# Codeuser0717/CVAE-GAN

Hardware: NVIDIA B200
Metric: train_samples_per_s (higher is better)
Workload: dtype f32

## Files before the change

cvae_gan_b200/csrc/api.cu:

```cuda
#include "engine.cuh"

namespace cvg {
const char* last_error();
int comm_unique_id(void* out128);
int comm_init(Engine& e, const void* id128, int rank, int world);
void comm_destroy(Engine& e);
}

using namespace cvg;

struct CvgHandle {
  Engine e;
};

#define H_OR_FAIL(h)                      \
  if (!(h)) {                             \
    cvg::set_error("null handle");        \
    return 1;                             \
  }


constexpr int FC_MAX_KC = 12;
template <int KC>
struct FcDispatch {
// ... 182 lines not shown

int cvg_nvl_local_handle(CvgHandle* h, void* out64) {
  H_OR_FAIL(h);
  if (!out64) CVG_FAIL("null argument");
  return nvl_local_handle(h->e, out64);
}
int cvg_nvl_attach(CvgHandle* h, const void* handles) {
  H_OR_FAIL(h);
  if (!handles) CVG_FAIL("null argument");
  return nvl_attach(h->e, handles);
}

int cvg_nvl_disable(CvgHandle* h) {
  H_OR_FAIL(h);
  nvl_destroy(h->e);
  return 0;
}

int cvg_step_d(CvgHandle* h, const float* x_real, int label, int B, const CvgNoise* noise, uint64_t seed,
               uint64_t counter, int flags, float* loss_out, void* stream) {
  H_OR_FAIL(h);
  if (!x_real) CVG_FAIL("null x_real");
  if (label < 0 || label >= h->e.K) CVG_FAIL("label out of range");
  StepRng rng;
  rng.seed = seed; rng.counter = counter;
  return step_d(h->e, x_real, label, B, noise, rng, flags, loss_out, (cudaStream_t)stream);
}
int cvg_step_c(CvgHandle* h, const float* x_real, int label, int B, const CvgNoise* noise, uint64_t seed,
               uint64_t counter, int flags, float* loss_out, void* stream) {
  H_OR_FAIL(h);
  if (!x_real) CVG_FAIL("null x_real");
  if (label < 0 || label >= h->e.K) CVG_FAIL("label out of range");
  StepRng rng;
  rng.seed = seed; rng.counter = counter;
  return step_c(h->e, x_real, label, B, noise, rng, flags, loss_out, (cudaStream_t)stream);
}
int cvg_step_g(CvgHandle* h, const float* x_real, int label, int B, const CvgNoise* noise, uint64_t seed,
               uint64_t counter, float lambda_class_now, int flags, float* loss_out, void* stream) {
  H_OR_FAIL(h);
  if (!x_real && !(flags & CVG_STEP_PRIOR_ONLY)) CVG_FAIL("null x_real");
  if ((flags & CVG_STEP_PRIOR_ONLY) && (flags & CVG_STEP_CVAE)) CVG_FAIL("CVG_STEP_PRIOR_ONLY and CVG_STEP_CVAE are mutually exclusive");
  if (label < 0 || label >= h->e.K) CVG_FAIL("label out of range");
  StepRng rng;
  rng.seed = seed; rng.counter = counter;
  rng.lambda_class = lambda_class_now; rng.lambda_nonzero = lambda_class_now != 0.f;
  return step_g(h->e, x_real, label, B, noise, rng, flags, loss_out, (cudaStream_t)stream);
}

int cvg_step_classifier(CvgHandle* h, const float* x, const int64_t* labels, int B, const CvgNoise* noise, uint64_t seed,
                        uint64_t counter, float lr, float beta1, float beta2, float eps, int flags, float* loss_out,
                        void* stream) {
  H_OR_FAIL(h);
  if (!x || !labels) CVG_FAIL("cvg_step_classifier: null argument");
  StepRng rng;
  rng.seed = seed; rng.counter = counter;
  AdamOverride ov{lr, beta1, beta2, eps};
  return step_classifier(h->e, x, (const long long*)labels, B, noise, rng, ov, flags, loss_out, (cudaStream_t)stream);
}

int cvg_visit(CvgHandle* h, int label, int B_local, int64_t B_global, const float* class_rows, int64_t n_rows,
              const float* x_batches, int d_loop, int c_loop, int g_loop, int flags, float* loss_out, void* stream) {
  H_OR_FAIL(h);
  if (label < 0 || label >= h->e.K) CVG_FAIL("label out of range");
  if (d_loop < 0 || c_loop < 0 || g_loop < 0) CVG_FAIL("cvg_visit: negative loop count");
  if ((flags & CVG_STEP_PRIOR_ONLY) && (flags & CVG_STEP_CVAE)) CVG_FAIL("CVG_STEP_PRIOR_ONLY and CVG_STEP_CVAE are mutually exclusive");
  if ((flags & CVG_STEP_CVAE) && d_loop != 0) CVG_FAIL("cvg_visit: a CVAE visit has no critic steps (d_loop must be 0, cvae.py:86-166)");
  return visit(h->e, label, B_local, B_global, class_rows, n_rows, x_batches, d_loop, c_loop, g_loop, flags, loss_out,
               (cudaStream_t)stream);
}

int cvg_ctl_set(CvgHandle* h, uint64_t seed, uint64_t counter, int set_rng, float lambda_class, int set_lambda, void* stream) {
  H_OR_FAIL(h);
  if (!h->e.ws_base) CVG_FAIL("workspace not bound");
  ctl_set_kernel<<<1, 32, 0, (cudaStream_t)stream>>>(h->e.ws.ctl, seed, counter, set_rng, lambda_class, set_lambda);
  CVG_CUDA(cudaGetLastError());
  h->e.launches++;
  return 0;
}

int cvg_adam(CvgHandle* h, int net_mask, void* stream) {
  H_OR_FAIL(h);
  return run_adam(h->e, net_mask, (cudaStream_t)stream);
}

int cvg_sample_rows(CvgHandle* h, const float* class_rows, int64_t n, int64_t B_global, int64_t draw_offset,
                    int B_local, uint64_t seed, uint64_t counter, float* x_out, int64_t* idx_out, void* stream) {
  H_OR_FAIL(h);
  if (!class_rows || !x_out || n < 1 || B_local < 1 || draw_offset < 0 || draw_offset + B_local > B_global)
    CVG_FAIL("cvg_sample_rows: bad argument");
  sample_rows_kernel<<<(B_local + 127) / 128, 128, 0, (cudaStream_t)stream>>>(
      class_rows, n, B_global, draw_offset, B_local, h->e.F, seed, counter, nullptr, 0, x_out, (long long*)idx_out);
  CVG_CUDA(cudaGetLastError());
  h->e.launches++;
  return 0;
}

int cvg_generate(CvgHandle* h, int label, int64_t n, const float* z, uint64_t seed, uint64_t row_offset, int train_mode,
                 float* x_out, void* stream) {
  H_OR_FAIL(h);
  if (n < 0 || (n > 0 && !x_out)) CVG_FAIL("cvg_generate: bad argument");
  return generate(h->e, label, n, z, seed, row_offset, train_mode, x_out, (cudaStream_t)stream);
}

int cvg_generate_filter(CvgHandle* h, int label, int64_t n, float thr, const float* z, uint64_t seed,
                        uint64_t row_offset, float* x_out, int64_t* idx_out, int64_t capacity,
                        unsigned long long* count_out, float* logits_out, uint8_t* keep_out, void* stream) {
  H_OR_FAIL(h);
  if (n < 0 || !count_out || (capacity > 0 && !x_out)) CVG_FAIL("cvg_generate_filter: bad argument");
  return generate_filter(h->e, label, n, thr, z, seed, row_offset, x_out, idx_out, capacity, count_out, logits_out,
                         keep_out, (cudaStream_t)stream);
}

int cvg_filter_logits(const float* logits, int64_t n, int K, int label, float thr, uint8_t* keep_out, void* stream) {
  if (!logits || !keep_out || n < 0) CVG_FAIL("cvg_filter_logits: bad argument");
  if (K < 1 || K > FILTER_MAXK) CVG_FAIL("cvg_filter_logits: K must be in [1, 32]");
  if (n == 0) return 0;
  filter_logits_kernel<<<(unsigned)((n + 255) / 256), 256, 0, (cudaStream_t)stream>>>(logits, n, K, label, thr, keep_out);
  CVG_CUDA(cudaGetLastError());
  return 0;
}

int cvg_filter_compact(const float* x, const float* logits, int64_t n, int F, int K, int label, float thr,
                       uint64_t row_offset, float* x_out, int64_t* idx_out, int64_t capacity,
                       unsigned long long* count_out, void* stream) {
  if (!x || !logits || !count_out || n < 0) CVG_FAIL("cvg_filter_compact: bad argument");
  if (K < 1 || K > FILTER_MAXK) CVG_FAIL("cvg_filter_compact: K must be in [1, 32]");
  if (n == 0) return 0;
  if (K > FC_MAX_KC) {
    filter_compact_kernel<false><<<(unsigned)((n + 255) / 256), 256, 0, (cudaStream_t)stream>>>(
        x, logits, n, 0, F, K, label, thr, row_offset, x_out, (long long*)idx_out, capacity, count_out, nullptr, nullptr);
  } else {
    const size_t smem = (size_t)FC_SUB_ROWS * K * sizeof(float);
    static int sms = 0;
    if (!sms) {
      int dev = 0;
      CVG_CUDA(cudaGetDevice(&dev));
      CVG_CUDA(cudaDeviceGetAttribute(&sms, cudaDevAttrMultiProcessorCount, dev));
      CVG_TRY(fc_set_attributes());
    }
    const long long slots = (long long)sms * 6;
    long long done = 0;
    while (done < n) {
      const long long left = n - done;
      const long long nblk1k = (left + FC_SUB_ROWS - 1) / FC_SUB_ROWS;
      const long long grid = nblk1k < slots ? nblk1k : slots;
      long long nsub = (nblk1k + grid - 1) / grid;
      long long rows_now = left;
      if (nsub > FC_MAXSUB) {
        nsub = FC_MAXSUB;
        rows_now = grid * nsub * FC_SUB_ROWS;
      }
      CVG_TRY(fc_launch(K, (unsigned)grid, smem, (cudaStream_t)stream, x + done * F, logits + done * K, rows_now, F, label, thr,
                        row_offset + (uint64_t)done, (int)nsub, x_out, (long long*)idx_out, capacity, count_out));
      CVG_CUDA(cudaGetLastError());
      done += rows_now;
    }
  }
  CVG_CUDA(cudaGetLastError());
  return 0;
}

int cvg_classifier_forward(CvgHandle* h, const float* x, int64_t n, float* logits_out, void* stream) {
  H_OR_FAIL(h);
  if (!x || !logits_out || n < 0) CVG_FAIL("cvg_classifier_forward: bad argument");
  return classifier_forward(h->e, x, n, logits_out, (cudaStream_t)stream);
}
int cvg_encoder_forward(CvgHandle* h, const float* x, int label, int64_t n, float* mu_out, float* logvar_out,
                        void* stream) {
  H_OR_FAIL(h);
  if (!x || !mu_out || !logvar_out || n < 0) CVG_FAIL("cvg_encoder_forward: bad argument");
  return encoder_forward(h->e, x, label, n, mu_out, logvar_out, (cudaStream_t)stream);
}

int cvg_patience_scan(const uint8_t* keep, int64_t n, int64_t num, int chunk, int patience, int64_t* rows_consumed,
                      int64_t* rows_accepted) {
  if (!keep || !rows_consumed || !rows_accepted || chunk < 1) CVG_FAIL("cvg_patience_scan: bad argument");
  int64_t pos = 0, got = 0;
  while (got < num && patience > 0) {
    const int64_t c = (num - got) < chunk ? (num - got) : chunk;
    if (pos + c > n) CVG_FAIL("cvg_patience_scan: row stream too short");
    int64_t k = 0;
    for (int64_t i = 0; i < c; ++i) k += keep[pos + i] ? 1 : 0;
    pos += c;
    got += k;
    if (k == 0) --patience;
  }
  *rows_consumed = pos;
  *rows_accepted = got;
  return 0;
}

int cvg_debug_read(CvgHandle* h, const char* name, int pass, int rows, float* dst, int* features_out, void* stream) {
  H_OR_FAIL(h);
  if (!name) CVG_FAIL("null name");
  Engine& e = h->e;
  const Workspace& w = e.ws;
  if (!e.ws_base) CVG_FAIL("workspace not bound");
  const std::string n(name);
  const float* p = nullptr;
  int C = 0;
  auto idx = [&](const char* prefix) -> int {
    const size_t L = strlen(prefix);
    if (n.size() == L + 1 && n.compare(0, L, prefix) == 0 && n[L] >= '0' && n[L] <= '2') return n[L] - '0';
    return -1;
  };
  int i;
  if (n == "xT") { p = w.xT; C = e.F; }
  else if (n == "z") { p = w.z; C = e.Z; }
  else if ((i = idx("g_h")) >= 0) { p = w.g_h[i]; C = e.gh[i]; }
  else if ((i = idx("g_dy")) >= 0) { p = w.g_dy[i]; C = e.gh[i]; }
  else if (n == "g_out") { p = w.g_out; C = e.F; }
  else if (n == "g_dout") { p = w.g_dout; C = e.F; }
  else if ((i = idx("e_h")) >= 0) { p = w.e_h[i]; C = e.eh[i]; }
  else if ((i = idx("e_dy")) >= 0) { p = w.e_dy[i]; C = e.eh[i]; }
  else if (n == "e_ml") { p = w.e_ml; C = 2 * e.Z; }
  else if (n == "e_dml") { p = w.e_dml; C = 2 * e.Z; }
  else if ((i = idx("d_a")) >= 0) { p = w.d_a[i]; C = e.dh[i]; }
  else if ((i = idx("d_g")) >= 0) { p = w.d_g[i]; C = e.dh[i]; }
  else if (n == "d_s") { p = w.d_s; C = 1; }
  else if (n == "c_a1") { p = w.c_a1; C = e.ch[0]; }
  else if (n == "c_h2") { p = w.c_h2; C = e.ch[1]; }
  else if (n == "c_a2") { p = w.c_a2; C = e.ch[1]; }
  else if (n == "c_a3") { p = w.c_a3; C = e.ch[2]; }
  else if (n == "c_logit") { p = w.c_logit; C = e.K; }
  else if (n == "c_dlogit") { p = w.c_dlogit; C = e.K; }
  else if ((i = idx("c_g")) >= 0) { p = w.c_g[i]; C = e.ch[i]; }
  else if (n == "dx") { p = w.dx; C = e.F; }
  else CVG_FAIL("cvg_debug_read: unknown buffer name");
  if (features_out) *features_out = C;
  if (!dst) return 0;
  if (rows < 1 || rows > w.ld || pass < 0 || pass > 1) CVG_FAIL("cvg_debug_read: bad rows/pass");
  to_row_major_kernel<<<(rows + 127) / 128, 128, 0, (cudaStream_t)stream>>>(p + (size_t)pass * C * w.ld, rows, C, w.ld, dst);
  CVG_CUDA(cudaGetLastError());
  return 0;
}

int cvg_debug_tc_counters(CvgHandle* h, long long* dev_counters) {
  H_OR_FAIL(h);
  h->e.tc_dbg = dev_counters;
  return 0;
}

int cvg_profile_enable(CvgHandle* h, int enable) {
  H_OR_FAIL(h);
  Engine& e = h->e;
  for (auto& r : e.prof_recs) {
    cudaEventDestroy(r.a);
    cudaEventDestroy(r.b);
  }
  e.prof_recs.clear();
  e.prof = enable != 0;
  return 0;
}

int cvg_profile_read(CvgHandle* h, int kernel_class, int64_t* launches, double* flops, double* ms) {
  H_OR_FAIL(h);
  if (!launches || !flops || !ms) CVG_FAIL("cvg_profile_read: null argument");
  Engine& e = h->e;
  *launches = 0;
  *flops = 0.0;
  *ms = 0.0;
  for (auto& r : e.prof_recs) {
    if (r.cls != kernel_class) continue;
    CVG_CUDA(cudaEventSynchronize(r.b));
    float t = 0.f;
    CVG_CUDA(cudaEventElapsedTime(&t, r.a, r.b));
    *launches += 1;
    *flops += r.flops;
    *ms += (double)t;
  }
  return 0;
}

int64_t cvg_launch_count(const CvgHandle* h) { return h ? h->e.launches : -1; }

int cvg_debug_set(CvgHandle* h, const char* key, int value) {
  H_OR_FAIL(h);
  if (!key) CVG_FAIL("null key");
  Engine& e = h->e;
  const std::string k(key);
  if (k == "train_mode") {
    if (value && !mk_supported(e)) CVG_FAIL("cvg_debug_set: the step-program kernel does not cover these layer widths");
    e.mk.enabled = value != 0;
  } else if (k == "mk_max_ops") e.mk.max_ops = value;
  else if (k == "mk_allbar") e.mk.allbar = value != 0;
  else if (k == "mk_coop") e.mk.coop = value != 0;
  else if (k == "hoist") e.hoist = value != 0;
  else if (k == "streams") e.ms.on = value != 0;
  else if (k == "chain") e.chain = value != 0;
  else if (k == "eg_split") e.eg_split = value != 0;
  else if (k == "fuse_stats") e.nvl.fuse = value != 0;
  else CVG_FAIL("cvg_debug_set: unknown key");
  return 0;
}

int cvg_debug_get(const CvgHandle* h, const char* key, int* value) {
  H_OR_FAIL(h);
  if (!key || !value) CVG_FAIL("null argument");
  const Engine& e = h->e;
  const std::string k(key);
  if (k == "train_mode") *value = e.mk.enabled ? 1 : 0;
  else if (k == "mk_last_nops") *value = e.mk.last_nops;
  else if (k == "mk_supported") *value = mk_supported(e) ? 1 : 0;
  else CVG_FAIL("cvg_debug_get: unknown key");
  return 0;
}

int cvg_debug_mk_cycles(CvgHandle* h, long long* out, int capacity, int* count) {
  H_OR_FAIL(h);
  Engine& e = h->e;
  if (!e.ws_base) CVG_FAIL("workspace not bound");
  const int n = e.mk.last_nops < capacity ? e.mk.last_nops : capacity;
  if (count) *count = n;
  if (out && n > 0) CVG_CUDA(cudaMemcpy(out, e.ws.mk_dbg, sizeof(long long) * n, cudaMemcpyDeviceToHost));
  if (out && capacity >= 2048 + 64 && n <= 1024) {
    CVG_CUDA(cudaMemcpy(out + 1024, e.ws.mk_dbg + 1024, sizeof(long long) * n, cudaMemcpyDeviceToHost));
    if (capacity >= 4096)
      for (int i = 0; i < n && i < (int)e.mk.last_kinds.size(); ++i) out[3072 + i] = e.mk.last_kinds[i];
  }
  if (out && capacity >= 2048 + 64) CVG_CUDA(cudaMemcpy(out + 2048, e.ws.mk_dbg + 2048, sizeof(long long) * 64, cudaMemcpyDeviceToHost));
  return 0;
}

}
```

cvae_gan_b200/csrc/chain.cuh:

```cuda
#pragma once
#include "gemm.cuh"
#include "misc_kernels.cuh"

namespace cvg {

constexpr int CH_TM = 32;
constexpr int CH_THREADS = 256;
constexpr int CH_NB = 64;
constexpr int CH_KC = 64;
constexpr int CH_H0 = 256, CH_H1 = 128, CH_H2 = 64;
constexpr int CH_MAX_IN = 256;
constexpr int CH_MAX_K = 32;
constexpr int CH_WBUF = 2 * CH_KC * CH_NB;

struct CriticChainArgs {
  int M = 0, ld = 0, F = 0;
  const float* x = nullptr;
  long long sx = 0;
  const float* W[4] = {};
  int ldw[4] = {};
  const float* b[4] = {};
  const float* wlabel = nullptr;
  int ldwl = 0;
  const float* inv_sigma = nullptr;
  const uint8_t* m1 = nullptr;
  const uint8_t* m2 = nullptr;
  float keep_inv = 1.f, slope = 0.2f;
  float* a[3] = {};
  float* s = nullptr;
  float* g[3] = {};
  double* osum = nullptr;
  float seed[2] = {0.f, 0.f};
};

struct ClassifierChainArgs {
  int M = 0, ld = 0, F = 0, K = 0, label = 0;
  const float* x = nullptr;
  long long sx = 0;
  const float* W[4] = {};
  const float* b[4] = {};
  const float* gamma = nullptr;
  const float* beta = nullptr;
  float ln_eps = 1e-5f;
  const uint8_t* m1 = nullptr;
  const uint8_t* m2 = nullptr;
  float keep_inv = 1.f;
  float *a1 = nullptr, *h2 = nullptr, *a2 = nullptr, *rs = nullptr, *a3 = nullptr, *logit = nullptr, *dlogit = nullptr;
  float* g[3] = {};
  float coef = 1.f;
  double* loss = nullptr;
  float* dgamma = nullptr;
  float* dbeta = nullptr;
  unsigned long long* acc = nullptr;
  unsigned* cnt = nullptr;
};

template <bool WT, class Ep>
__device__ __forceinline__ void chain_layer(const float* X, const float* __restrict__ W, int ldw, int R, int N, float* wbuf,
                                            Ep ep) {
  const int tid = threadIdx.x;
  const int grp = tid >> 6, t64 = tid & 63;
  const int tm = (t64 & 7) * 4, tn = (t64 >> 3) * 8;
  const int Rp = (R + TBK - 1) / TBK * TBK;
  const int nkc = (Rp + CH_KC - 1) / CH_KC;
  const bool wvec = (ldw & 3) == 0;
  for (int n0 = 0; n0 < N; n0 += CH_NB) {
    float4 pre[4];
    auto gload = [&](int kc) {
#pragma unroll
      for (int j = 0; j < 4; ++j) pre[j] = make_float4(0.f, 0.f, 0.f, 0.f);
      if (WT) {
        const int n = n0 + (tid & 63);
        if (n >= N) return;
#pragma unroll
        for (int j = 0; j < 4; ++j) {
          const int k = kc + (tid >> 6) * 16 + 4 * j;
          const float* src = W + (size_t)n * ldw + k;
          if (wvec && k + 3 < R) {
            pre[j] = ld4(src);
          } else {
            if (k < R) pre[j].x = src[0];
            if (k + 1 < R) pre[j].y = src[1];
            if (k + 2 < R) pre[j].z = src[2];
            if (k + 3 < R) pre[j].w = src[3];
          }
        }
      } else {
        const int k = kc + (tid >> 2);
        if (k >= R) return;
#pragma unroll
        for (int j = 0; j < 4; ++j) {
          const int n = n0 + (tid & 3) * 16 + 4 * j;
          const float* src = W + (size_t)k * ldw + n;
          if (wvec && n + 3 < N) {
            pre[j] = ld4(src);
          } else {
            if (n < N) pre[j].x = src[0];
            if (n + 1 < N) pre[j].y = src[1];
            if (n + 2 < N) pre[j].z = src[2];
            if (n + 3 < N) pre[j].w = src[3];
          }
        }
      }
    };
    auto sstore = [&](float* buf) {
      if (WT) {
        const int kq = (tid >> 6) * 16, n = tid & 63;
#pragma unroll
        for (int j = 0; j < 4; ++j) {
          buf[(kq + 4 * j + 0) * CH_NB + n] = pre[j].x;
          buf[(kq + 4 * j + 1) * CH_NB + n] = pre[j].y;
          buf[(kq + 4 * j + 2) * CH_NB + n] = pre[j].z;
          buf[(kq + 4 * j + 3) * CH_NB + n] = pre[j].w;
        }
      } else {
#pragma unroll
        for (int j = 0; j < 4; ++j) st4(buf + (tid >> 2) * CH_NB + (tid & 3) * 16 + 4 * j, pre[j]);
      }
    };
    float acc[4][8];
#pragma unroll
    for (int i = 0; i < 4; ++i)
#pragma unroll
      for (int j = 0; j < 8; ++j) acc[i][j] = 0.f;
    gload(0);
    sstore(wbuf);
    __syncthreads();
    for (int c = 0; c < nkc; ++c) {
      const float* cur = wbuf + (c & 1) * CH_KC * CH_NB;
      const int kc = c * CH_KC;
      if (c + 1 < nkc) gload(kc + CH_KC);
      const int nt = min(CH_KC, Rp - kc) / TBK;
      for (int t = 0; t < nt; ++t) {
#pragma unroll
        for (int q = 0; q < 4; ++q) {
          const int kl = t * TBK + grp * 4 + q;
          const float4 a = ld4(X + (size_t)(kc + kl) * CH_TM + tm);
          const float4 w0 = ld4(cur + kl * CH_NB + tn), w1 = ld4(cur + kl * CH_NB + tn + 4);
          const float av[4] = {a.x, a.y, a.z, a.w};
          const float wv[8] = {w0.x, w0.y, w0.z, w0.w, w1.x, w1.y, w1.z, w1.w};
#pragma unroll
          for (int i = 0; i < 4; ++i)
#pragma unroll
            for (int j = 0; j < 8; ++j) acc[i][j] = fmaf(av[i], wv[j], acc[i][j]);
        }
      }
      if (c + 1 < nkc) sstore(wbuf + ((c + 1) & 1) * CH_KC * CH_NB);
      __syncthreads();
    }
    float* red = wbuf;
#pragma unroll
    for (int j = 0; j < 8; ++j)
      st4(red + ((size_t)grp * CH_NB + tn + j) * CH_TM + tm, make_float4(acc[0][j], acc[1][j], acc[2][j], acc[3][j]));
    __syncthreads();
    {
      const int n = tid >> 2;
#pragma unroll
      for (int h = 0; h < 2; ++h) {
        const int m = (tid & 3) * 8 + 4 * h;
        const float4 y = ksum4(ld4(red + ((size_t)0 * CH_NB + n) * CH_TM + m), ld4(red + ((size_t)1 * CH_NB + n) * CH_TM + m),
                               ld4(red + ((size_t)2 * CH_NB + n) * CH_TM + m), ld4(red + ((size_t)3 * CH_NB + n) * CH_TM + m));
        if (n0 + n < N) ep(n0 + n, m, y);
      }
    }
    __syncthreads();
  }
}

struct FwdEp {
  const float* bias;
  const float* wlabel;
  int ldwl;
  float scale;
  int act;
  float slope;
  const uint8_t* mask;
  float keep_inv;
  float* Y;
  float* S;
  int ld, m0, M;
  __device__ __forceinline__ double operator()(int n, int m, float4 v) const {
    float y[4] = {v.x, v.y, v.z, v.w};
    const float b = ep_bias(bias, wlabel, ldwl, n, scale);
#pragma unroll
    for (int i = 0; i < 4; ++i) y[i] = ep_act(ep_linear(y[i], scale, b), act, slope);
    const size_t off = (size_t)n * ld + m0 + m;
    if (mask) {
      const uchar4 mk = *reinterpret_cast<const uchar4*>(mask + off);
      y[0] = ep_dropout(y[0], mk.x, keep_inv);
      y[1] = ep_dropout(y[1], mk.y, keep_inv);
      y[2] = ep_dropout(y[2], mk.z, keep_inv);
      y[3] = ep_dropout(y[3], mk.w, keep_inv);
    }
    st4(Y + off, make_float4(y[0], y[1], y[2], y[3]));
    double tot = 0.0;
#pragma unroll
    for (int i = 0; i < 4; ++i) {
      const bool valid = m0 + m + i < M;
      if (S) S[n * CH_TM + m + i] = valid ? y[i] : 0.f;
      if (valid) tot += (double)y[i];
    }
    return tot;
  }
};

struct DactEp {
  float scale;
  const uint8_t* mask;
  float keep_inv;
  float neg;
  const float* A;
  float* Y;
  float* S;
  int ld, m0, M;
  __device__ __forceinline__ void operator()(int n, int m, float4 v) const {
    float y[4] = {v.x, v.y, v.z, v.w};
    const size_t off = (size_t)n * ld + m0 + m;
    float keep[4] = {1.f, 1.f, 1.f, 1.f};
    if (mask) {
      const uchar4 mk = *reinterpret_cast<const uchar4*>(mask + off);
      keep[0] = ep_keep(mk.x, keep_inv);
      keep[1] = ep_keep(mk.y, keep_inv);
      keep[2] = ep_keep(mk.z, keep_inv);
      keep[3] = ep_keep(mk.w, keep_inv);
    }
#pragma unroll
    for (int i = 0; i < 4; ++i) y[i] = ep_dact(y[i], scale, keep[i], A[n * CH_TM + m + i], neg);
    st4(Y + off, make_float4(y[0], y[1], y[2], y[3]));
    if (S)
#pragma unroll
      for (int i = 0; i < 4; ++i) S[n * CH_TM + m + i] = m0 + m + i < M ? y[i] : 0.f;
  }
};

__device__ __forceinline__ void chain_stage(float* S, int rows, const float* src, int nvalid, int ld, int m0, int M) {
  for (int i = threadIdx.x; i < rows * CH_TM; i += CH_THREADS) {
    const int k = i / CH_TM, m = i % CH_TM;
    S[i] = (k < nvalid && m0 + m < M) ? src[(size_t)k * ld + m0 + m] : 0.f;
  }
}

__host__ __device__ inline int chain_x_rows(int F, int K) {
  const int fp = (F + TBK - 1) / TBK * TBK;
  const int kp = 2 * ((K + TBK - 1) / TBK * TBK);
  return fp > kp ? fp : kp;
}
inline size_t critic_chain_smem(int F) {
  return sizeof(float) * ((size_t)CH_WBUF + (size_t)(CH_H0 + CH_H1 + CH_H2) * CH_TM + (size_t)chain_x_rows(F, 1) * CH_TM);
}
inline size_t classifier_chain_smem(int F, int K) {
  return sizeof(float) * ((size_t)CH_WBUF + (size_t)(CH_H0 + 2 * CH_H1 + CH_H2) * CH_TM + (size_t)chain_x_rows(F, K) * CH_TM);
}

__global__ void __launch_bounds__(CH_THREADS, 2) critic_chain_kernel(const CriticChainArgs g) {
  extern __shared__ __align__(16) float ch_smem[];
  float* wbuf = ch_smem;
  float* A0 = wbuf + CH_WBUF;
  float* A1 = A0 + CH_H0 * CH_TM;
  float* A2 = A1 + CH_H1 * CH_TM;
  float* X = A2 + CH_H2 * CH_TM;
  const int pass = blockIdx.y, m0 = blockIdx.x * CH_TM;
  const int M = g.M, ld = g.ld;
  const size_t ps0 = (size_t)pass * CH_H0 * ld, ps1 = (size_t)pass * CH_H1 * ld, ps2 = (size_t)pass * CH_H2 * ld;

  chain_stage(X, (g.F + TBK - 1) / TBK * TBK, g.x + (long long)pass * g.sx, g.F, ld, m0, M);
  __syncthreads();
  chain_layer<true>(X, g.W[0], g.ldw[0], g.F, CH_H0, wbuf,
                    FwdEp{g.b[0], g.wlabel, g.ldwl, g.inv_sigma[0 + pass], ACT_LRELU, g.slope, g.m1 + ps0, g.keep_inv,
                          g.a[0] + ps0, A0, ld, m0, M});
  chain_layer<true>(A0, g.W[1], g.ldw[1], CH_H0, CH_H1, wbuf,
                    FwdEp{g.b[1], nullptr, 0, g.inv_sigma[2 + pass], ACT_LRELU, g.slope, g.m2 + ps1, g.keep_inv,
                          g.a[1] + ps1, A1, ld, m0, M});
  chain_layer<true>(A1, g.W[2], g.ldw[2], CH_H1, CH_H2, wbuf,
                    FwdEp{g.b[2], nullptr, 0, g.inv_sigma[4 + pass], ACT_LRELU, g.slope, nullptr, 1.f,
                          g.a[2] + ps2, A2, ld, m0, M});
  double tot = 0.0;
  const FwdEp score{g.b[3], nullptr, 0, g.inv_sigma[6 + pass], ACT_NONE, g.slope, nullptr, 1.f,
                    g.s + (size_t)pass * ld, nullptr, ld, m0, M};
  chain_layer<true>(A2, g.W[3], g.ldw[3], CH_H2, 1, wbuf, [&](int n, int m, float4 y) { tot += score(n, m, y); });
  tot = warp_sum_d(tot);
  if (threadIdx.x == 0) atomicAdd(g.osum + pass, tot);
  for (int i = threadIdx.x; i < TBK * CH_TM; i += CH_THREADS)
    X[i] = (i < CH_TM && m0 + i < M) ? g.seed[pass] : 0.f;
  __syncthreads();
  chain_layer<false>(X, g.W[3], g.ldw[3], 1, CH_H2, wbuf,
                     DactEp{g.inv_sigma[6 + pass], nullptr, 1.f, g.slope, A2, g.g[2] + ps2, A2, ld, m0, M});
  chain_layer<false>(A2, g.W[2], g.ldw[2], CH_H2, CH_H1, wbuf,
                     DactEp{g.inv_sigma[4 + pass], g.m2 + ps1, g.keep_inv, g.slope, A1, g.g[1] + ps1, A1, ld, m0, M});
  chain_layer<false>(A1, g.W[1], g.ldw[1], CH_H1, CH_H0, wbuf,
                     DactEp{g.inv_sigma[2 + pass], g.m1 + ps0, g.keep_inv, g.slope, A0, g.g[0] + ps0, nullptr, ld, m0, M});
}

__global__ void __launch_bounds__(CH_THREADS, 2) classifier_chain_kernel(const ClassifierChainArgs g) {
  extern __shared__ __align__(16) float ch_smem[];
  __shared__ float red1[8][LN_ROWS], red2[8][LN_ROWS];
  __shared__ unsigned s_last;
  float* wbuf = ch_smem;
  float* A1 = wbuf + CH_WBUF;
  float* H2 = A1 + CH_H0 * CH_TM;
  float* A2 = H2 + CH_H1 * CH_TM;
  float* A3 = A2 + CH_H1 * CH_TM;
  float* X = A3 + CH_H2 * CH_TM;
  const int Kp = (g.K + TBK - 1) / TBK * TBK;
  float* L = X;
  float* D = X + Kp * CH_TM;
  const int pass = blockIdx.y, m0 = blockIdx.x * CH_TM;
  const int M = g.M, ld = g.ld;
  const int lane = threadIdx.x & 31, w = threadIdx.x >> 5;
  const bool valid = m0 + lane < M;
  const size_t ps0 = (size_t)pass * CH_H0 * ld, ps1 = (size_t)pass * CH_H1 * ld, ps2 = (size_t)pass * CH_H2 * ld;
  const size_t psk = (size_t)pass * g.K * ld;

  chain_stage(X, (g.F + TBK - 1) / TBK * TBK, g.x + (long long)pass * g.sx, g.F, ld, m0, M);
  for (int i = threadIdx.x; i < CH_H1 * CH_TM; i += CH_THREADS) A2[i] = 0.f;
  __syncthreads();
  chain_layer<true>(X, g.W[0], g.F, g.F, CH_H0, wbuf,
                    FwdEp{g.b[0], nullptr, 0, 1.0f, ACT_RELU, 0.f, g.m1 + ps0, g.keep_inv, g.a1 + ps0, A1, ld, m0, M});
  chain_layer<true>(A1, g.W[1], CH_H0, CH_H0, CH_H1, wbuf,
                    FwdEp{g.b[1], nullptr, 0, 1.0f, ACT_NONE, 0.f, nullptr, 1.f, g.h2 + ps1, H2, ld, m0, M});
  float mean, rstd;
  {
    const uint8_t* mk = g.m2 + ps1 + m0 + lane;
    float* a2g = g.a2 + ps1 + m0 + lane;
    ln_fwd_row<LN_MAXF>(
        CH_H1, valid, g.ln_eps, g.gamma, g.beta, mk, ld, g.keep_inv, red1, [&](int c) { return H2[c * CH_TM + lane]; },
        [&](int c, float n) {
          a2g[(size_t)c * ld] = n;
          A2[c * CH_TM + lane] = n;
        },
        mean, rstd);
    if (valid && w == 0) {
      float* rs = g.rs + (size_t)pass * 2 * ld;
      rs[m0 + lane] = mean;
      rs[ld + m0 + lane] = rstd;
    }
  }
  for (int i = threadIdx.x; i < Kp * CH_TM; i += CH_THREADS) D[i] = 0.f;
  __syncthreads();
  chain_layer<true>(A2, g.W[2], CH_H1, CH_H1, CH_H2, wbuf,
                    FwdEp{g.b[2], nullptr, 0, 1.0f, ACT_RELU, 0.f, nullptr, 1.f, g.a3 + ps2, A3, ld, m0, M});
  chain_layer<true>(A3, g.W[3], CH_H2, CH_H2, g.K, wbuf,
                    FwdEp{g.b[3], nullptr, 0, 1.0f, ACT_NONE, 0.f, nullptr, 1.f, g.logit + psk, L, ld, m0, M});
  if (w == 0) {
    double nll = 0.0;
    if (valid) {
      nll = ce_row(L + lane, CH_TM, D + lane, CH_TM, g.K, g.label, g.coef);
      float* dg = g.dlogit + psk + m0 + lane;
      for (int k = 0; k < g.K; ++k) dg[(size_t)k * ld] = D[k * CH_TM + lane];
    }
    nll = warp_sum_d(nll);
    if (lane == 0 && nll != 0.0) atomicAdd(g.loss + pass, nll);
  }
  __syncthreads();
  chain_layer<false>(D, g.W[3], CH_H2, g.K, CH_H2, wbuf,
                     DactEp{1.0f, nullptr, 1.f, 0.f, A3, g.g[2] + ps2, A3, ld, m0, M});
  chain_layer<false>(A3, g.W[2], CH_H1, CH_H2, CH_H1, wbuf,
                     DactEp{1.0f, g.m2 + ps1, g.keep_inv, 0.f, A2, g.g[1] + ps1, A2, ld, m0, M});
  {
    float* dhg = g.g[1] + ps1 + m0 + lane;
    ln_bwd_row<LN_MAXF>(
        CH_H1, valid, mean, rstd, g.gamma, red1, red2, [&](int c) { return A2[c * CH_TM + lane]; },
        [&](int c) { return H2[c * CH_TM + lane]; },
        [&](int c, float v) {
          dhg[(size_t)c * ld] = v;
          A2[c * CH_TM + lane] = v;
        },
        g.dgamma ? g.acc : nullptr);
  }
  if (g.dgamma) {
    __threadfence();
    __syncthreads();
    if (threadIdx.x == 0) s_last = atomicAdd(g.cnt, 1u) == gridDim.x * gridDim.y - 1 ? 1u : 0u;
    __syncthreads();
    if (s_last) {
      __threadfence();
      for (int e = threadIdx.x; e < 2 * CH_H1; e += CH_THREADS) {
        const float v = det_unfix(__ldcg(g.acc + e));
        g.acc[e] = 0ull;
        atomicAdd(e < CH_H1 ? g.dgamma + e : g.dbeta + (e - CH_H1), v);
      }
      if (threadIdx.x == 0) *g.cnt = 0u;
    }
  }
  __syncthreads();
  chain_layer<false>(A2, g.W[1], CH_H0, CH_H1, CH_H0, wbuf,
                     DactEp{1.0f, g.m1 + ps0, g.keep_inv, 0.f, A1, g.g[0] + ps0, nullptr, ld, m0, M});
}

}
```

Before: 13.77 million.

## Stream chain weights through a cross-layer cp.async ring with warp-shuffle reduction

Replaces the per-layer double-buffered register-staged weight loads in the critic and classifier chain kernels with a 4-stage cp.async ring buffer. The ring follows a per-block layer schedule, so prefetch of the next layer's weights overlaps the current layer's compute and epilogue. The shared-memory cross-group reduction is replaced by warp shuffles, with transposed and swizzled smem layouts and dropout masks prefetched before the k-loop. It also adds debug queries for occupancy; the change adds complexity and may alter register pressure and occupancy.

```diff
diff --git a/cvae_gan_b200/csrc/api.cu b/cvae_gan_b200/csrc/api.cu
--- a/cvae_gan_b200/csrc/api.cu
+++ b/cvae_gan_b200/csrc/api.cu
@@ -508,6 +508,11 @@
   if (k == "train_mode") *value = e.mk.enabled ? 1 : 0;
   else if (k == "mk_last_nops") *value = e.mk.last_nops;
   else if (k == "mk_supported") *value = mk_supported(e) ? 1 : 0;
+  else if (k == "critic_chain_ctas_per_sm")
+    CVG_CUDA(cudaOccupancyMaxActiveBlocksPerMultiprocessor(value, critic_chain_kernel, CH_THREADS, critic_chain_smem(e.F)));
+  else if (k == "classifier_chain_ctas_per_sm")
+    CVG_CUDA(cudaOccupancyMaxActiveBlocksPerMultiprocessor(value, classifier_chain_kernel, CH_THREADS,
+                                                           classifier_chain_smem(e.F, e.K)));
   else CVG_FAIL("cvg_debug_get: unknown key");
   return 0;
 }
diff --git a/cvae_gan_b200/csrc/chain.cuh b/cvae_gan_b200/csrc/chain.cuh
--- a/cvae_gan_b200/csrc/chain.cuh
+++ b/cvae_gan_b200/csrc/chain.cuh
@@ -7,11 +7,13 @@
 constexpr int CH_TM = 32;
 constexpr int CH_THREADS = 256;
 constexpr int CH_NB = 64;
-constexpr int CH_KC = 64;
+constexpr int CH_KS = 32;
+constexpr int CH_STAGES = 4;
 constexpr int CH_H0 = 256, CH_H1 = 128, CH_H2 = 64;
 constexpr int CH_MAX_IN = 256;
 constexpr int CH_MAX_K = 32;
-constexpr int CH_WBUF = 2 * CH_KC * CH_NB;
+constexpr int CH_SLOT = CH_KS * CH_NB;
+constexpr int CH_WBUF = CH_STAGES * CH_SLOT;
 
 struct CriticChainArgs {
   int M = 0, ld = 0, F = 0;
@@ -55,116 +57,182 @@
   unsigned* cnt = nullptr;
 };
 
-template <bool WT, class Ep>
-__device__ __forceinline__ void chain_layer(const float* X, const float* __restrict__ W, int ldw, int R, int N, float* wbuf,
-                                            Ep ep) {
-  const int tid = threadIdx.x;
-  const int grp = tid >> 6, t64 = tid & 63;
-  const int tm = (t64 & 7) * 4, tn = (t64 >> 3) * 8;
-  const int Rp = (R + TBK - 1) / TBK * TBK;
-  const int nkc = (Rp + CH_KC - 1) / CH_KC;
-  const bool wvec = (ldw & 3) == 0;
-  for (int n0 = 0; n0 < N; n0 += CH_NB) {
-    float4 pre[4];
-    auto gload = [&](int kc) {
-#pragma unroll
-      for (int j = 0; j < 4; ++j) pre[j] = make_float4(0.f, 0.f, 0.f, 0.f);
-      if (WT) {
-        const int n = n0 + (tid & 63);
-        if (n >= N) return;
-#pragma unroll
-        for (int j = 0; j < 4; ++j) {
-          const int k = kc + (tid >> 6) * 16 + 4 * j;
-          const float* src = W + (size_t)n * ldw + k;
-          if (wvec && k + 3 < R) {
-            pre[j] = ld4(src);
-          } else {
-            if (k < R) pre[j].x = src[0];
-            if (k + 1 < R) pre[j].y = src[1];
-            if (k + 2 < R) pre[j].z = src[2];
-            if (k + 3 < R) pre[j].w = src[3];
+struct ChLayer {
+  const float* W;
+  int ldw, R, N;
+  int wt;
+  int vec;
+};
+
+__device__ __forceinline__ void cp_async4(float* dst, const float* src, int bytes) {
+  asm volatile("cp.async.ca.shared.global [%0], [%1], 4, %2;\n" ::"r"((unsigned)__cvta_generic_to_shared(dst)), "l"(src),
+               "r"(bytes));
+}
+__device__ __forceinline__ void cp_async16(float* dst, const float* src, int bytes) {
+  asm volatile("cp.async.cg.shared.global [%0], [%1], 16, %2;\n" ::"r"((unsigned)__cvta_generic_to_shared(dst)), "l"(src),
+               "r"(bytes));
+}
+__device__ __forceinline__ void cp_async_commit() { asm volatile("cp.async.commit_group;\n" ::); }
+template <int N>
+__device__ __forceinline__ void cp_async_wait() { asm volatile("cp.async.wait_group %0;\n" ::"n"(N)); }
+
+__device__ __forceinline__ int ch_rpad(int R) { return (R + TBK - 1) / TBK * TBK; }
+
+struct ChRing {
+  float* buf;
+  const ChLayer* L;
+  int nl;
+  int cl;
+  int pl, pn0, pkc;
+  int pi, ci;
+
+  __device__ __forceinline__ void issue() {
+    if (pl < nl) {
+      const ChLayer d = L[pl];
+      const int kn = min(CH_KS, ch_rpad(d.R) - pkc);
+      const int ksh = kn == CH_KS ? 5 : 4;
+      float* dst = buf + (pi & (CH_STAGES - 1)) * CH_SLOT;
+      if (d.wt) {
+        if (d.vec) {
+          for (int i = threadIdx.x; i < (CH_NB * kn) >> 2; i += CH_THREADS) {
+            const int n = i >> (ksh - 2), k = (i & ((kn >> 2) - 1)) * 4;
+            const int gk = pkc + k, gn = pn0 + n;
+            const int bytes = gn < d.N ? 4 * max(0, min(4, d.R - gk)) : 0;
+            cp_async16(dst + n * CH_KS + k, bytes ? d.W + (size_t)gn * d.ldw + gk : d.W, bytes);
+          }
+        } else {
+          for (int i = threadIdx.x; i < CH_NB * kn; i += CH_THREADS) {
+            const int n = i >> ksh, k = i & (kn - 1);
+            const int gk = pkc + k, gn = pn0 + n;
+            const bool ok = gn < d.N && gk < d.R;
+            cp_async4(dst + n * CH_KS + k, ok ? d.W + (size_t)gn * d.ldw + gk : d.W, ok ? 4 : 0);
           }
         }
       } else {
-        const int k = kc + (tid >> 2);
-        if (k >= R) return;
-#pragma unroll
-        for (int j = 0; j < 4; ++j) {
-          const int n = n0 + (tid & 3) * 16 + 4 * j;
-          const float* src = W + (size_t)k * ldw + n;
-          if (wvec && n + 3 < N) {
-            pre[j] = ld4(src);
-          } else {
-            if (n < N) pre[j].x = src[0];
-            if (n + 1 < N) pre[j].y = src[1];
-            if (n + 2 < N) pre[j].z = src[2];
-            if (n + 3 < N) pre[j].w = src[3];
+        if (d.vec) {
+          for (int i = threadIdx.x; i < kn * (CH_NB / 4); i += CH_THREADS) {
+            const int k = i >> 4, n = (i & 15) * 4;
+            const int gk = pkc + k, gn = pn0 + n;
+            const int bytes = gk < d.R ? 4 * max(0, min(4, d.N - gn)) : 0;
+            cp_async16(dst + k * CH_NB + (n ^ (((k >> 2) & 3) << 3)), bytes ? d.W + (size_t)gk * d.ldw + gn : d.W, bytes);
+          }
+        } else {
+          for (int i = threadIdx.x; i < kn * CH_NB; i += CH_THREADS) {
+            const int k = i >> 6, n = i & (CH_NB - 1);
+            const int gk = pkc + k, gn = pn0 + n;
+            const bool ok = gk < d.R && gn < d.N;
+            cp_async4(dst + k * CH_NB + (n ^ (((k >> 2) & 3) << 3)), ok ? d.W + (size_t)gk * d.ldw + gn : d.W, ok ? 4 : 0);
           }
         }
       }
-    };
-    auto sstore = [&](float* buf) {
-      if (WT) {
-        const int kq = (tid >> 6) * 16, n = tid & 63;
-#pragma unroll
-        for (int j = 0; j < 4; ++j) {
-          buf[(kq + 4 * j + 0) * CH_NB + n] = pre[j].x;
-          buf[(kq + 4 * j + 1) * CH_NB + n] = pre[j].y;
-          buf[(kq + 4 * j + 2) * CH_NB + n] = pre[j].z;
-          buf[(kq + 4 * j + 3) * CH_NB + n] = pre[j].w;
-        }
-      } else {
-#pragma unroll
-        for (int j = 0; j < 4; ++j) st4(buf + (tid >> 2) * CH_NB + (tid & 3) * 16 + 4 * j, pre[j]);
-      }
-    };
-    float acc[4][8];
-#pragma unroll
-    for (int i = 0; i < 4; ++i)
-#pragma unroll
-      for (int j = 0; j < 8; ++j) acc[i][j] = 0.f;
-    gload(0);
-    sstore(wbuf);
-    __syncthreads();
-    for (int c = 0; c < nkc; ++c) {
-      const float* cur = wbuf + (c & 1) * CH_KC * CH_NB;
-      const int kc = c * CH_KC;
-      if (c + 1 < nkc) gload(kc + CH_KC);
-      const int nt = min(CH_KC, Rp - kc) / TBK;
-      for (int t = 0; t < nt; ++t) {
-#pragma unroll
-        for (int q = 0; q < 4; ++q) {
-          const int kl = t * TBK + grp * 4 + q;
-          const float4 a = ld4(X + (size_t)(kc + kl) * CH_TM + tm);
-          const float4 w0 = ld4(cur + kl * CH_NB + tn), w1 = ld4(cur + kl * CH_NB + tn + 4);
-          const float av[4] = {a.x, a.y, a.z, a.w};
-          const float wv[8] = {w0.x, w0.y, w0.z, w0.w, w1.x, w1.y, w1.z, w1.w};
-#pragma unroll
-          for (int i = 0; i < 4; ++i)
-#pragma unroll
-            for (int j = 0; j < 8; ++j) acc[i][j] = fmaf(av[i], wv[j], acc[i][j]);
+      pkc += CH_KS;
+      if (pkc >= ch_rpad(d.R)) {
+        pkc = 0;
+        pn0 += CH_NB;
+        if (pn0 >= d.N) {
+          pn0 = 0;
+          ++pl;
         }
       }
-      if (c + 1 < nkc) sstore(wbuf + ((c + 1) & 1) * CH_KC * CH_NB);
-      __syncthreads();
-    }
-    float* red = wbuf;
-#pragma unroll
-    for (int j = 0; j < 8; ++j)
-      st4(red + ((size_t)grp * CH_NB + tn + j) * CH_TM + tm, make_float4(acc[0][j], acc[1][j], acc[2][j], acc[3][j]));
+    }
+    cp_async_commit();
+    ++pi;
+  }
+  __device__ __forceinline__ void start(float* b, const ChLayer* l, int n) {
+    buf = b; L = l; nl = n; cl = 0;
+    pl = pn0 = pkc = 0; pi = ci = 0;
+#pragma unroll 1
+    for (int s = 0; s < CH_STAGES - 1; ++s) issue();
+  }
+  __device__ __forceinline__ const float* acquire() {
+    cp_async_wait<CH_STAGES - 2>();
     __syncthreads();
-    {
-      const int n = tid >> 2;
-#pragma unroll
-      for (int h = 0; h < 2; ++h) {
-        const int m = (tid & 3) * 8 + 4 * h;
-        const float4 y = ksum4(ld4(red + ((size_t)0 * CH_NB + n) * CH_TM + m), ld4(red + ((size_t)1 * CH_NB + n) * CH_TM + m),
-                               ld4(red + ((size_t)2 * CH_NB + n) * CH_TM + m), ld4(red + ((size_t)3 * CH_NB + n) * CH_TM + m));
-        if (n0 + n < N) ep(n0 + n, m, y);
+    issue();
+    return buf + (ci++ & (CH_STAGES - 1)) * CH_SLOT;
+  }
+};
+
+__device__ __forceinline__ float ch_sel4(int c, float v0, float v1, float v2, float v3) {
+  return c == 0 ? v0 : c == 1 ? v1 : c == 2 ? v2 : v3;
+}
+
+template <bool WT, class Ep>
+__device__ __forceinline__ void chain_layer(const float* X, ChRing& rg, Ep ep) {
+  const ChLayer& d = rg.L[rg.cl];
+  const int R = d.R, N = d.N;
+  const int lane = threadIdx.x & 31, g = lane >> 3;
+  const int tm = (lane & 7) * 4, tn = (threadIdx.x >> 5) * 8;
+  const int Rp = ch_rpad(R);
+#pragma unroll 1
+  for (int n0 = 0; n0 < N; n0 += CH_NB) {
+    const int nl = n0 + tn + 2 * g;
+    uchar4 mk[2];
+#pragma unroll
+    for (int e = 0; e < 2; ++e) mk[e] = nl + e < N ? ep.mask_at(nl + e, tm) : make_uchar4(1, 1, 1, 1);
+    float acc[4][8];
+#pragma unroll
+    for (int i = 0; i < 4; ++i)
+#pragma unroll
+      for (int j = 0; j < 8; ++j) acc[i][j] = 0.f;
+#pragma unroll 1
+    for (int kc = 0; kc < Rp; kc += CH_KS) {
+      const float* cur = rg.acquire();
+      const int nt = min(CH_KS, Rp - kc) / TBK;
+#pragma unroll 1
+      for (int t = 0; t < nt; ++t) {
+        const int kl = t * TBK + g * 4;
+        float4 a[4];
+#pragma unroll
+        for (int q = 0; q < 4; ++q) a[q] = ld4(X + (size_t)(kc + kl + q) * CH_TM + tm);
+        if (WT) {
+          float4 w[8];
+#pragma unroll
+          for (int j = 0; j < 8; ++j) w[j] = ld4(cur + (tn + j) * CH_KS + kl);
+#pragma unroll
+          for (int q = 0; q < 4; ++q) {
+            const float av[4] = {a[q].x, a[q].y, a[q].z, a[q].w};
+#pragma unroll
+            for (int j = 0; j < 8; ++j) {
+              const float wv = q == 0 ? w[j].x : q == 1 ? w[j].y : q == 2 ? w[j].z : w[j].w;
+#pragma unroll
+              for (int i = 0; i < 4; ++i) acc[i][j] = fmaf(av[i], wv, acc[i][j]);
+            }
+          }
+        } else {
+#pragma unroll
+          for (int q = 0; q < 4; ++q) {
+            const float* row = cur + (kl + q) * CH_NB;
+            const float4 w0 = ld4(row + (tn ^ (g << 3))), w1 = ld4(row + ((tn + 4) ^ (g << 3)));
+            const float av[4] = {a[q].x, a[q].y, a[q].z, a[q].w};
+            const float wv[8] = {w0.x, w0.y, w0.z, w0.w, w1.x, w1.y, w1.z, w1.w};
+#pragma unroll
+            for (int i = 0; i < 4; ++i)
+#pragma unroll
+              for (int j = 0; j < 8; ++j) acc[i][j] = fmaf(av[i], wv[j], acc[i][j]);
+          }
+        }
       }
     }
-    __syncthreads();
-  }
+    float y[8];
+#pragma unroll
+    for (int v = 0; v < 8; ++v) {
+      const int i = v >> 1, e = v & 1;
+      float pr[4];
+      pr[0] = ch_sel4(g, acc[i][e], acc[i][2 + e], acc[i][4 + e], acc[i][6 + e]);
+#pragma unroll
+      for (int r = 1; r < 4; ++r)
+        pr[r] = __shfl_xor_sync(0xffffffffu, ch_sel4(g ^ r, acc[i][e], acc[i][2 + e], acc[i][4 + e], acc[i][6 + e]), r << 3);
+      const float p01 = g < 2 ? pr[0] + pr[1] : pr[2] + pr[3];
+      const float p2 = g == 0 ? pr[2] : g == 1 ? pr[3] : g == 2 ? pr[0] : pr[1];
+      const float p3 = g == 0 ? pr[3] : g == 1 ? pr[2] : g == 2 ? pr[1] : pr[0];
+      y[v] = (p01 + p2) + p3;
+    }
+#pragma unroll
+    for (int e = 0; e < 2; ++e)
+      if (nl + e < N) ep(nl + e, tm, make_float4(y[e], y[2 + e], y[4 + e], y[6 + e]), mk[e]);
+  }
+  ++rg.cl;
+  __syncthreads();
 }
 
 struct FwdEp {
@@ -179,14 +247,16 @@
   float* Y;
   float* S;
   int ld, m0, M;
-  __device__ __forceinline__ double operator()(int n, int m, float4 v) const {
+  __device__ __forceinline__ uchar4 mask_at(int n, int m) const {
+    return mask ? *reinterpret_cast<const uchar4*>(mask + (size_t)n * ld + m0 + m) : make_uchar4(1, 1, 1, 1);
+  }
+  __device__ __forceinline__ double operator()(int n, int m, float4 v, uchar4 mk) const {
     float y[4] = {v.x, v.y, v.z, v.w};
     const float b = ep_bias(bias, wlabel, ldwl, n, scale);
 #pragma unroll
     for (int i = 0; i < 4; ++i) y[i] = ep_act(ep_linear(y[i], scale, b), act, slope);
     const size_t off = (size_t)n * ld + m0 + m;
     if (mask) {
-      const uchar4 mk = *reinterpret_cast<const uchar4*>(mask + off);
       y[0] = ep_dropout(y[0], mk.x, keep_inv);
       y[1] = ep_dropout(y[1], mk.y, keep_inv);
       y[2] = ep_dropout(y[2], mk.z, keep_inv);
@@ -196,10 +266,13 @@
     double tot = 0.0;
 #pragma unroll
     for (int i = 0; i < 4; ++i) {
-      const bool valid = m0 + m + i < M;
-      if (S) S[n * CH_TM + m + i] = valid ? y[i] : 0.f;
-      if (valid) tot += (double)y[i];
-    }
+      if (m0 + m + i < M) {
+        tot += (double)y[i];
+      } else {
+        y[i] = 0.f;
+      }
+    }
+    if (S) st4(S + n * CH_TM + m, make_float4(y[0], y[1], y[2], y[3]));
     return tot;
   }
 };
@@ -213,25 +286,40 @@
   float* Y;
   float* S;
   int ld, m0, M;
-  __device__ __forceinline__ void operator()(int n, int m, float4 v) const {
+  __device__ __forceinline__ uchar4 mask_at(int n, int m) const {
+    return mask ? *reinterpret_cast<const uchar4*>(mask + (size_t)n * ld + m0 + m) : make_uchar4(1, 1, 1, 1);
+  }
+  __device__ __forceinline__ void operator()(int n, int m, float4 v, uchar4 mk) const {
     float y[4] = {v.x, v.y, v.z, v.w};
     const size_t off = (size_t)n * ld + m0 + m;
     float keep[4] = {1.f, 1.f, 1.f, 1.f};
     if (mask) {
-      const uchar4 mk = *reinterpret_cast<const uchar4*>(mask + off);
       keep[0] = ep_keep(mk.x, keep_inv);
       keep[1] = ep_keep(mk.y, keep_inv);
       keep[2] = ep_keep(mk.z, keep_inv);
       keep[3] = ep_keep(mk.w, keep_inv);
     }
-#pragma unroll
-    for (int i = 0; i < 4; ++i) y[i] = ep_dact(y[i], scale, keep[i], A[n * CH_TM + m + i], neg);
+    const float4 a = ld4(A + n * CH_TM + m);
+    const float av[4] = {a.x, a.y, a.z, a.w};
+#pragma unroll
+    for (int i = 0; i < 4; ++i) y[i] = ep_dact(y[i], scale, keep[i], av[i], neg);
     st4(Y + off, make_float4(y[0], y[1], y[2], y[3]));
     if (S)
-#pragma unroll
-      for (int i = 0; i < 4; ++i) S[n * CH_TM + m + i] = m0 + m + i < M ? y[i] : 0.f;
-  }
-};
+      st4(S + n * CH_TM + m, make_float4(m0 + m < M ? y[0] : 0.f, m0 + m + 1 < M ? y[1] : 0.f, m0 + m + 2 < M ? y[2] : 0.f,
+                                         m0 + m + 3 < M ? y[3] : 0.f));
+  }
+};
+
+struct SumEp {
+  FwdEp f;
+  double* tot;
+  __device__ __forceinline__ uchar4 mask_at(int n, int m) const { return f.mask_at(n, m); }
+  __device__ __forceinline__ void operator()(int n, int m, float4 v, uchar4 mk) const { *tot += f(n, m, v, mk); }
+};
+
+__device__ __forceinline__ ChLayer ch_sched(const float* W, int ldw, int R, int N, bool wt) {
+  return ChLayer{W, ldw, R, N, wt ? 1 : 0, (ldw & 3) == 0 && ((size_t)W & 15) == 0};
+}
 
 __device__ __forceinline__ void chain_stage(float* S, int rows, const float* src, int nvalid, int ld, int m0, int M) {
   for (int i = threadIdx.x; i < rows * CH_TM; i += CH_THREADS) {
@@ -262,32 +350,45 @@
   const int pass = blockIdx.y, m0 = blockIdx.x * CH_TM;
   const int M = g.M, ld = g.ld;
   const size_t ps0 = (size_t)pass * CH_H0 * ld, ps1 = (size_t)pass * CH_H1 * ld, ps2 = (size_t)pass * CH_H2 * ld;
-
+  __shared__ ChLayer sched[7];
+
+  if (threadIdx.x == 0) {
+    sched[0] = ch_sched(g.W[0], g.ldw[0], g.F, CH_H0, true);
+    sched[1] = ch_sched(g.W[1], g.ldw[1], CH_H0, CH_H1, true);
+    sched[2] = ch_sched(g.W[2], g.ldw[2], CH_H1, CH_H2, true);
+    sched[3] = ch_sched(g.W[3], g.ldw[3], CH_H2, 1, true);
+    sched[4] = ch_sched(g.W[3], g.ldw[3], 1, CH_H2, false);
+    sched[5] = ch_sched(g.W[2], g.ldw[2], CH_H2, CH_H1, false);
+    sched[6] = ch_sched(g.W[1], g.ldw[1], CH_H1, CH_H0, false);
+  }
+  __syncthreads();
+  ChRing rg;
+  rg.start(wbuf, sched, 7);
   chain_stage(X, (g.F + TBK - 1) / TBK * TBK, g.x + (long long)pass * g.sx, g.F, ld, m0, M);
   __syncthreads();
-  chain_layer<true>(X, g.W[0], g.ldw[0], g.F, CH_H0, wbuf,
+  chain_layer<true>(X, rg,
                     FwdEp{g.b[0], g.wlabel, g.ldwl, g.inv_sigma[0 + pass], ACT_LRELU, g.slope, g.m1 + ps0, g.keep_inv,
                           g.a[0] + ps0, A0, ld, m0, M});
-  chain_layer<true>(A0, g.W[1], g.ldw[1], CH_H0, CH_H1, wbuf,
+  chain_layer<true>(A0, rg,
                     FwdEp{g.b[1], nullptr, 0, g.inv_sigma[2 + pass], ACT_LRELU, g.slope, g.m2 + ps1, g.keep_inv,
                           g.a[1] + ps1, A1, ld, m0, M});
-  chain_layer<true>(A1, g.W[2], g.ldw[2], CH_H1, CH_H2, wbuf,
+  chain_layer<true>(A1, rg,
                     FwdEp{g.b[2], nullptr, 0, g.inv_sigma[4 + pass], ACT_LRELU, g.slope, nullptr, 1.f,
                           g.a[2] + ps2, A2, ld, m0, M});
   double tot = 0.0;
   const FwdEp score{g.b[3], nullptr, 0, g.inv_sigma[6 + pass], ACT_NONE, g.slope, nullptr, 1.f,
                     g.s + (size_t)pass * ld, nullptr, ld, m0, M};
-  chain_layer<true>(A2, g.W[3], g.ldw[3], CH_H2, 1, wbuf, [&](int n, int m, float4 y) { tot += score(n, m, y); });
+  chain_layer<true>(A2, rg, SumEp{score, &tot});
   tot = warp_sum_d(tot);
   if (threadIdx.x == 0) atomicAdd(g.osum + pass, tot);
   for (int i = threadIdx.x; i < TBK * CH_TM; i += CH_THREADS)
     X[i] = (i < CH_TM && m0 + i < M) ? g.seed[pass] : 0.f;
   __syncthreads();
-  chain_layer<false>(X, g.W[3], g.ldw[3], 1, CH_H2, wbuf,
+  chain_layer<false>(X, rg,
                      DactEp{g.inv_sigma[6 + pass], nullptr, 1.f, g.slope, A2, g.g[2] + ps2, A2, ld, m0, M});
-  chain_layer<false>(A2, g.W[2], g.ldw[2], CH_H2, CH_H1, wbuf,
+  chain_layer<false>(A2, rg,
                      DactEp{g.inv_sigma[4 + pass], g.m2 + ps1, g.keep_inv, g.slope, A1, g.g[1] + ps1, A1, ld, m0, M});
-  chain_layer<false>(A1, g.W[1], g.ldw[1], CH_H1, CH_H0, wbuf,
+  chain_layer<false>(A1, rg,
                      DactEp{g.inv_sigma[2 + pass], g.m1 + ps0, g.keep_inv, g.slope, A0, g.g[0] + ps0, nullptr, ld, m0, M});
 }
 
@@ -310,13 +411,26 @@
   const bool valid = m0 + lane < M;
   const size_t ps0 = (size_t)pass * CH_H0 * ld, ps1 = (size_t)pass * CH_H1 * ld, ps2 = (size_t)pass * CH_H2 * ld;
   const size_t psk = (size_t)pass * g.K * ld;
-
+  __shared__ ChLayer sched[7];
+
+  if (threadIdx.x == 0) {
+    sched[0] = ch_sched(g.W[0], g.F, g.F, CH_H0, true);
+    sched[1] = ch_sched(g.W[1], CH_H0, CH_H0, CH_H1, true);
+    sched[2] = ch_sched(g.W[2], CH_H1, CH_H1, CH_H2, true);
+    sched[3] = ch_sched(g.W[3], CH_H2, CH_H2, g.K, true);
+    sched[4] = ch_sched(g.W[3], CH_H2, g.K, CH_H2, false);
+    sched[5] = ch_sched(g.W[2], CH_H1, CH_H2, CH_H1, false);
+    sched[6] = ch_sched(g.W[1], CH_H0, CH_H1, CH_H0, false);
+  }
+  __syncthreads();
+  ChRing rg;
+  rg.start(wbuf, sched, 7);
   chain_stage(X, (g.F + TBK - 1) / TBK * TBK, g.x + (long long)pass * g.sx, g.F, ld, m0, M);
   for (int i = threadIdx.x; i < CH_H1 * CH_TM; i += CH_THREADS) A2[i] = 0.f;
   __syncthreads();
-  chain_layer<true>(X, g.W[0], g.F, g.F, CH_H0, wbuf,
+  chain_layer<true>(X, rg,
                     FwdEp{g.b[0], nullptr, 0, 1.0f, ACT_RELU, 0.f, g.m1 + ps0, g.keep_inv, g.a1 + ps0, A1, ld, m0, M});
-  chain_layer<true>(A1, g.W[1], CH_H0, CH_H0, CH_H1, wbuf,
+  chain_layer<true>(A1, rg,
                     FwdEp{g.b[1], nullptr, 0, 1.0f, ACT_NONE, 0.f, nullptr, 1.f, g.h2 + ps1, H2, ld, m0, M});
   float mean, rstd;
   {
@@ -337,9 +451,9 @@
   }
   for (int i = threadIdx.x; i < Kp * CH_TM; i += CH_THREADS) D[i] = 0.f;
   __syncthreads();
-  chain_layer<true>(A2, g.W[2], CH_H1, CH_H1, CH_H2, wbuf,
+  chain_layer<true>(A2, rg,
                     FwdEp{g.b[2], nullptr, 0, 1.0f, ACT_RELU, 0.f, nullptr, 1.f, g.a3 + ps2, A3, ld, m0, M});
-  chain_layer<true>(A3, g.W[3], CH_H2, CH_H2, g.K, wbuf,
+  chain_layer<true>(A3, rg,
                     FwdEp{g.b[3], nullptr, 0, 1.0f, ACT_NONE, 0.f, nullptr, 1.f, g.logit + psk, L, ld, m0, M});
   if (w == 0) {
     double nll = 0.0;
@@ -352,9 +466,9 @@
     if (lane == 0 && nll != 0.0) atomicAdd(g.loss + pass, nll);
   }
   __syncthreads();
-  chain_layer<false>(D, g.W[3], CH_H2, g.K, CH_H2, wbuf,
+  chain_layer<false>(D, rg,
                      DactEp{1.0f, nullptr, 1.f, 0.f, A3, g.g[2] + ps2, A3, ld, m0, M});
-  chain_layer<false>(A3, g.W[2], CH_H1, CH_H2, CH_H1, wbuf,
+  chain_layer<false>(A3, rg,
                      DactEp{1.0f, g.m2 + ps1, g.keep_inv, 0.f, A2, g.g[1] + ps1, A2, ld, m0, M});
   {
     float* dhg = g.g[1] + ps1 + m0 + lane;
@@ -383,7 +497,7 @@
     }
   }
   __syncthreads();
-  chain_layer<false>(A2, g.W[1], CH_H0, CH_H1, CH_H0, wbuf,
+  chain_layer<false>(A2, rg,
                      DactEp{1.0f, g.m1 + ps0, g.keep_inv, 0.f, A1, g.g[0] + ps0, nullptr, ld, m0, M});
 }
 
```

Result: slower. 12.62 million (median of 6 runs) (-8.4%).
